# pynbody/topsy

Hardware: AMD Instinct MI355X
Metric: particles/sec splatted to 1024^2 buffer (higher is better)
Workload: dtype f32

## Files before the change

### topsy_amd/csrc/tsp_api.hip

```cpp
#include <stdarg.h>
#include <string.h>

#include <algorithm>
#include <vector>

#include "tsp_internal.h"

namespace tsp {

static thread_local char g_err[1024] = "";

void set_error(const char *fmt, ...) {
    va_list ap;
    va_start(ap, fmt);
    vsnprintf(g_err, sizeof(g_err), fmt, ap);
    va_end(ap);
}

int ensure_array(float **p, int64_t n) {
    if (*p) {
        TSP_HIP(hipFree(*p));
        *p = nullptr;
    }
    if (n > 0) TSP_HIP(hipMalloc((void **)p, (size_t)n * sizeof(float)));
// ... 644 lines not shown
int tsp_content_values(tsp_context *ctx, const int64_t *ranks, int n_ranks, float *out) {
    TSP_REQUIRE(ctx && ranks && out && n_ranks >= 0, TSP_EINVAL, "bad argument");
    TSP_REQUIRE(ctx->sort_keys_alt, TSP_ESTATE, "tsp_content_sort has not been called");
    TSP_HIP(hipSetDevice(ctx->device));
    for (int i = 0; i < n_ranks; ++i) {
        TSP_REQUIRE(ranks[i] >= 0 && ranks[i] < ctx->sorted_count, TSP_EINVAL, "rank %lld outside [0, %lld)",
                    (long long)ranks[i], (long long)ctx->sorted_count);
        uint32_t key;
        TSP_HIP(hipMemcpy(&key, ctx->sort_keys_alt + ranks[i], 4, hipMemcpyDeviceToHost));
        const uint32_t bits = (key & 0x80000000u) ? (key & 0x7fffffffu) : ~key;
        memcpy(&out[i], &bits, 4);
    }
    return TSP_OK;
}

int tsp_get_stats(tsp_context *ctx, tsp_stats *out) {
    TSP_REQUIRE(ctx && out, TSP_EINVAL, "NULL argument");
    *out = ctx->stats;
    return TSP_OK;
}

int tsp_set_option(tsp_context *ctx, const char *name, int64_t value) {
    TSP_REQUIRE(ctx && name, TSP_EINVAL, "NULL argument");
    if (!strcmp(name, "count_fragments")) {
        ctx->count_fragments = value != 0;
        return TSP_OK;
    }
    if (!strcmp(name, "p_small_milli")) {
        TSP_REQUIRE(value >= 0 && value <= 16000, TSP_EINVAL, "p_small out of range (kernel S packs <= 16 texel columns per footprint)");
        ctx->p_small = (float)value * 1e-3f;
        return TSP_OK;
    }
    if (!strcmp(name, "debug_no_raster")) {
        ctx->debug_no_raster = value != 0;
        return TSP_OK;
    }
    if (!strcmp(name, "huge_split") || !strcmp(name, "stream_blocks_per_cu")) {
        TSP_REQUIRE(value >= 0 && value <= 4096, TSP_EINVAL, "%s out of range", name);
        if (name[0] == 'h') ctx->huge_split = (int)value;
        else ctx->stream_blocks_per_cu = (int)value;
        return TSP_OK;
    }
    if (!strcmp(name, "slice_records")) {
        TSP_REQUIRE(value == 0 || (value >= 64 && value <= (1ll << 27)), TSP_EINVAL, "%s: 0 or 64 .. 2^27", name);
        ctx->slice_records = value;
        return TSP_OK;
    }
    if (!strcmp(name, "debug_fail_stage")) {
        TSP_REQUIRE(value >= 0 && value <= 2, TSP_EINVAL, "%s out of range", name);
        ctx->debug_fail_stage = (int)value;
        return TSP_OK;
    }
    if (!strcmp(name, "debug_gather_full_lut")) { ctx->debug_gather_full_lut = value ? 1 : 0; return TSP_OK; }
    if (!strcmp(name, "mid_item_scale_milli")) {
        TSP_REQUIRE(value >= 1 && value <= 100000, TSP_EINVAL, "%s out of range", name);
        ctx->mid_item_scale = (double)value * 1e-3;
        return TSP_OK;
    }
    if (!strcmp(name, "mid_narrow_px_milli")) {
        TSP_REQUIRE(value >= 0 && value <= 64000, TSP_EINVAL, "%s out of range", name);
        ctx->mid_narrow_px = (float)value * 1e-3f;
        return TSP_OK;
    }
    if (!strcmp(name, "mid_item_records")) {
        TSP_REQUIRE(value == 0 || (value >= 64 && value <= 8192 && (value & (value - 1)) == 0), TSP_EINVAL, "%s: 0 or a power of two from 64 to 8192", name);
        ctx->mid_item_records = (int)value;
        return TSP_OK;
    }
    if (!strcmp(name, "stream_batch_chunks")) {
        TSP_REQUIRE(value >= 4 && value <= 4096, TSP_EINVAL, "%s out of range", name);
        ctx->stream_batch_chunks = (int)value;
        return TSP_OK;
    }
    if (!strcmp(name, "huge_band_mib")) {
        TSP_REQUIRE(value >= 0 && value <= (1 << 20), TSP_EINVAL, "%s out of range", name);
        ctx->huge_band_budget = value << 20;
        return TSP_OK;
    }
    if (!strcmp(name, "huge_variant")) {
        TSP_REQUIRE(value >= 1 && value <= 7 && value != 3, TSP_EINVAL, "huge_variant out of range");
        ctx->huge_variant = (int)value;
        return TSP_OK;
    }
    if (!strcmp(name, "reorder_interleave")) {
        TSP_REQUIRE(value >= 0 && value <= 2, TSP_EINVAL, "%s out of range", name);
        ctx->reorder_interleave = (int)value;
        return TSP_OK;
    }
    if (!strcmp(name, "chunk_cull")) {
        ctx->chunk_cull = value != 0;
        return TSP_OK;
    }
    if (!strcmp(name, "overlap_mid_huge")) {
        ctx->overlap_mid_huge = value != 0;
        return TSP_OK;
    }
    if (!strcmp(name, "use_quantity")) {
        ctx->use_quantity = value != 0;
        return TSP_OK;
    }
    if (!strcmp(name, "active_channels")) {
        TSP_REQUIRE((value == 2 || value == 4) && value <= ctx->Ccap, TSP_EINVAL, "bad channel count %lld", (long long)value);
        ctx->C = (int)value;
        return TSP_OK;
    }
    set_error("unknown option '%s'", name);
    return TSP_EINVAL;
}

int tsp_measure_read_bandwidth(tsp_context *ctx, int64_t bytes, int iters, double *gbps_out) {
    TSP_REQUIRE(ctx && gbps_out && bytes > 0 && iters > 0, TSP_EINVAL, "bad argument");
    TSP_HIP(hipSetDevice(ctx->device));
    return measure_read_bandwidth(ctx, bytes, iters, gbps_out);
}

}
```

### topsy_amd/csrc/tsp_gather.hip

```cpp
#include <algorithm>
#include <cmath>
#include <type_traits>

#include "tsp_pipeline.h"

namespace tsp {


template <int T> __device__ __forceinline__ void fmac_quad(float &acc, float rowval, float v) {
    static_assert(T >= 0 && T < 4, "quad lane");
    if (T == 0) asm volatile("v_fmac_f32_dpp %0, %1, %2 " TSP_DPP_QUAD(0) : "+v"(acc) : "v"(rowval), "v"(v));
    if (T == 1) asm volatile("v_fmac_f32_dpp %0, %1, %2 " TSP_DPP_QUAD(1) : "+v"(acc) : "v"(rowval), "v"(v));
    if (T == 2) asm volatile("v_fmac_f32_dpp %0, %1, %2 " TSP_DPP_QUAD(2) : "+v"(acc) : "v"(rowval), "v"(v));
    if (T == 3) asm volatile("v_fmac_f32_dpp %0, %1, %2 " TSP_DPP_QUAD(3) : "+v"(acc) : "v"(rowval), "v"(v));
}
template <int T> __device__ __forceinline__ float mul_quad(float rowval, float v) {
    float r;
    if (T == 0) asm volatile("v_mul_f32_dpp %0, %1, %2 " TSP_DPP_QUAD(0) : "=v"(r) : "v"(rowval), "v"(v));
    if (T == 1) asm volatile("v_mul_f32_dpp %0, %1, %2 " TSP_DPP_QUAD(1) : "=v"(r) : "v"(rowval), "v"(v));
    if (T == 2) asm volatile("v_mul_f32_dpp %0, %1, %2 " TSP_DPP_QUAD(2) : "=v"(r) : "v"(rowval), "v"(v));
    if (T == 3) asm volatile("v_mul_f32_dpp %0, %1, %2 " TSP_DPP_QUAD(3) : "=v"(r) : "v"(rowval), "v"(v));
    return r;
}
__device__ __forceinline__ void fmac_plain(float &acc, float x, float y) {
    asm volatile("v_fmac_f32_e32 %0, %1, %2" : "+v"(acc) : "v"(x), "v"(y));
}

constexpr int PT_ROWS = 66;
constexpr int PT_STRIDE = 65;

constexpr int H2T = 256;

template <int MODE, int NACC, int W, int HR, int OCC, bool CNT>
__global__ __launch_bounds__(H2T, OCC) void splat_huge2_kernel(TileArgs a) {
    constexpr int C = (MODE == TSP_MODE_RGB) ? 4 : 2;
    constexpr int NW = (MODE == TSP_MODE_RGB) ? 2 : 1;
    constexpr int TW = 2 * 64 * W, TH = 2 * HR;
    constexpr int NG = HR / 4;
    static_assert(HR == 16 || HR == 32 || HR == 64, "rows per wave strip");
    typedef typename std::conditional<HR == 64, unsigned long long, unsigned>::type mask_t;
    extern __shared__ __attribute__((aligned(16))) float smem[];
    float *PT = smem;
    float2 *rt_all = reinterpret_cast<float2 *>(smem + ((PT_ROWS * PT_STRIDE + 3) & ~3));

    const int tid = threadIdx.x, lane = tid & 63, wv = __builtin_amdgcn_readfirstlane(tid >> 6);
    const int R = a.cam.R;
    const int tile_id = blockIdx.x / a.split, sp = blockIdx.x % a.split;
    const int tx0 = (tile_id % a.tiles_x) * TW, ty0 = (tile_id / a.tiles_x) * TH;
    for (int i = tid; i < PT_ROWS * PT_STRIDE; i += H2T) {
        const int j = min(i / PT_STRIDE, 63), x = min(i % PT_STRIDE, 63);
        PT[i] = a.mips[j * 64 + x];
    }
    float2 *rt = rt_all + wv * 64;
    const float2 *rt_quad = rt + (lane & 3);
    const int sx = tx0 + 64 * W * (wv & 1), sy = ty0 + HR * (wv >> 1);
    const float sx0 = (float)sx, sx1 = (float)(sx + 64 * W), sy0 = (float)sy, sy1 = (float)(sy + HR);
    float pxc[W];
#pragma unroll
    for (int w = 0; w < W; ++w) pxc[w] = (sx + 64 * w + lane < R) ? (float)(sx + 64 * w + lane) + 0.5f : __builtin_inff();
    const int myrow = lane & (HR - 1);
    const float pyc_own = (sy + myrow < R) ? (float)(sy + myrow) + 0.5f : __builtin_inff();

    constexpr int FOLD_EVERY = TSP_FOLD_EVERY;
    float acc[HR * W][NACC];
#pragma unroll
    for (int p = 0; p < HR * W; ++p)
#pragma unroll
        for (int c = 0; c < NACC; ++c) acc[p][c] = 0.0f;
    unsigned long long n_frag = 0;
    const char *PTb = reinterpret_cast<const char *>(PT);
    __syncthreads();
    if (sx >= R || sy >= R) return;

    const float4 *geom = a.geom;
    const float *wts = a.w;
    unsigned n_rec = (unsigned)a.n_records;
    if (a.hband_count) {
        const int band = ty0 / HBAND_H;
        geom += (size_t)band * a.hband_stride;
        wts += (size_t)band * a.hband_stride * NW;
        n_rec = (unsigned)a.hband_count[band];
    }
    const unsigned n_runs = (n_rec + HDEAL - 1) / HDEAL, usplit = (unsigned)a.split, n_last = max(n_rec, 1u) - 1u;
    const unsigned lane_off = (unsigned)(lane / HDEAL) * usplit * HDEAL + (unsigned)(lane & (HDEAL - 1));
    auto batch_base = [&](unsigned run0) -> unsigned { return (run0 * usplit + sp) * HDEAL; };
    auto fetch = [&](unsigned run0, float4 &g, float &gw1, float &gw2) {
        const unsigned rc = min(batch_base(run0) + lane_off, n_last);
        g = geom[rc];
        gw1 = (NACC >= 2) ? wts[rc * NW] : 0.0f;
        gw2 = (NW == 2) ? wts[rc * NW + 1] : 0.0f;
    };
    float4 g_next; float gw1_next, gw2_next;
    fetch(0, g_next, gw1_next, gw2_next);
    __builtin_amdgcn_s_waitcnt(0x0F70);
    unsigned run0 = 0;
    do {
    int since_fold = 0;
    for (; run0 * usplit < n_runs && since_fold < FOLD_EVERY; run0 += 64 / HDEAL) {
        float4 g = g_next;
        const float gw1 = gw1_next, gw2 = gw2_next;
        if (batch_base(run0) + lane_off >= n_rec) g.z = 0.0f;
        fetch(run0 + 64 / HDEAL, g_next, gw1_next, gw2_next);
        const float g_half = 0.5f * g.z;
        bool hit;
        {
            const float sdx = fmaxf(fmaxf(sx0 - g.x, g.x - sx1), 0.0f), sdy = fmaxf(fmaxf(sy0 - g.y, g.y - sy1), 0.0f);
            hit = g.z > 0.0f && sdx < g_half && sdy < g_half && !(a.disc_k2 > 0.0f && sdx * sdx + sdy * sdy >= a.disc_k2 * g.z * g.z);
        }
        unsigned long long hits = __ballot(hit);
        if (hits == 0ull) continue;
        since_fold += __popcll(hits);
        const float g_invP = 1.0f / g.z;
        const float g_w1 = (MODE == TSP_MODE_RGB) ? gw1 : g.w * gw1;
        constexpr int NH = 64 / HR;
        while (hits) {
            int srcs[NH], n_h = 0;
#pragma unroll
            for (int i = 0; i < NH; ++i) {
                srcs[i] = i ? srcs[0] : 0;
                if (hits) { srcs[i] = __ffsll((long long)hits) - 1; hits &= hits - 1; n_h = i + 1; }
            }
            unsigned long long cov64, chg64, jmp64;
            int r512;
            {
                int src_l = srcs[0];
#pragma unroll
                for (int i = 1; i < NH; ++i) src_l = (lane >= HR * i) ? srcs[i] : src_l;
                const int bp = src_l << 2;
                const float pcy_l = __int_as_float(__builtin_amdgcn_ds_bpermute(bp, __float_as_int(g.y)));
                const float half_l = __int_as_float(__builtin_amdgcn_ds_bpermute(bp, __float_as_int(g_half)));
                const float invP_l = __int_as_float(__builtin_amdgcn_ds_bpermute(bp, __float_as_int(g_invP)));
                const float d = pyc_own - pcy_l;
                const float cv = (__builtin_fabsf(d) < half_l) ? 1.0f : 0.0f;
                const float v = (d + half_l) * invP_l;
                const float tv = __builtin_amdgcn_fmed3f(__builtin_fmaf(v, 64.0f, -0.5f), 0.0f, 63.0f);
                const float fr = __builtin_amdgcn_fractf(tv) * cv;
                const int r = (int)tv;
                const int rprev = __builtin_amdgcn_mov_dpp(r, 0x138, 0xf, 0xf, false);
                r512 = __mul24(r, PT_STRIDE * 4);
                asm volatile("" ::: "memory");
                rt[lane] = make_float2(fr, cv - fr);
                asm volatile("" ::: "memory");
                constexpr unsigned long long ROW0S = (HR == 64) ? 1ull : ((HR == 32) ? 0x0000000100000001ull : 0x0001000100010001ull);
                cov64 = __builtin_amdgcn_fcmpf(__builtin_fabsf(d), half_l, 4 );
                chg64 = __builtin_amdgcn_uicmp((unsigned)r, (unsigned)rprev, 33 ) & cov64 & ~ROW0S;
                jmp64 = __builtin_amdgcn_uicmp((unsigned)r, (unsigned)(rprev + 1), 33 ) & chg64;
            }
            for (int hh = 0; hh < n_h; ++hh) {
            int src = srcs[0];
#pragma unroll
            for (int i = 1; i < NH; ++i) src = (hh == i) ? srcs[i] : src;
            constexpr unsigned long long ROWS = (HR == 64) ? ~0ull : ((1ull << (HR & 63)) - 1ull);
            mask_t covmask = (mask_t)((cov64 >> ((HR * hh) & 63)) & ROWS), chgmask = (mask_t)((chg64 >> ((HR * hh) & 63)) & ROWS),
                   jmpmask = (mask_t)((jmp64 >> ((HR * hh) & 63)) & ROWS);
            const float pcx = __int_as_float(__builtin_amdgcn_readlane(__float_as_int(g.x), src));
            const float half = __int_as_float(__builtin_amdgcn_readlane(__float_as_int(g_half), src));
            const float invP = __int_as_float(__builtin_amdgcn_readlane(__float_as_int(g_invP), src));
            float4 wq;
            wq.x = __int_as_float(__builtin_amdgcn_readlane(__float_as_int(g.w), src));
            wq.y = (NACC >= 2) ? __int_as_float(__builtin_amdgcn_readlane(__float_as_int(g_w1), src)) : 0.0f;
            wq.z = (NACC >= 3) ? __int_as_float(__builtin_amdgcn_readlane(__float_as_int(gw2), src)) : 0.0f;
            wq.w = 0.0f;
            if (NACC >= 2) {
                asm volatile("v_mov_b32 %0, %1" : "=v"(wq.x) : "s"(wq.x));
                asm volatile("v_mov_b32 %0, %1" : "=v"(wq.y) : "s"(wq.y));
                if (NACC >= 3) asm volatile("v_mov_b32 %0, %1" : "=v"(wq.z) : "s"(wq.z));
            }
            const float2 *rt_quad_h = rt_quad + HR * hh;
            if (covmask == 0) continue;
            const mask_t first = covmask & ((mask_t)0 - covmask);
            chgmask &= ~first; jmpmask &= ~first;
            constexpr bool JIT = (HR >= 32);
            constexpr int NRF = JIT ? 2 : NG;
            float2 rowf[NRF];
            if constexpr (JIT) rowf[0] = rt_quad_h[0];
            else {
#pragma unroll
                for (int k = 0; k < NG; ++k) rowf[k] = rt_quad_h[4 * k];
            }
            int caddr[W];
            float fxs[W], gxs[W];
            int ncov_x = 0;
#pragma unroll
            for (int w = 0; w < W; ++w) {
                const float d = pxc[w] - pcx;
                const bool covered = __builtin_fabsf(d) < half;
                const float u = (d + half) * invP;
                const float tu = __builtin_amdgcn_fmed3f(__builtin_fmaf(u, 64.0f, -0.5f), 0.0f, 63.0f);
                caddr[w] = ((int)tu) * 4;
                const float cw = covered ? ((NACC == 1) ? wq.x : 1.0f) : 0.0f;
                const float fr = __builtin_amdgcn_fractf(tu);
                fxs[w] = fr * cw;
                gxs[w] = (1.0f - fr) * cw;
                if (CNT) ncov_x += covered ? 1 : 0;
            }
            float top[W], bot[W];
            float2 nxt[W];
            auto pair_at = [&](int w, int byteoff) -> float2 {
                const float *t = reinterpret_cast<const float *>(PTb + byteoff + caddr[w]);
                return make_float2(t[0], t[1]);
            };
            auto lerp = [&](int w, float2 t) -> float { return __builtin_fmaf(t.y, fxs[w], t.x * gxs[w]); };
            int r_off = __builtin_amdgcn_readlane(r512, (HR == 64 ? __ffsll((long long)covmask) : __ffs((int)covmask)) - 1 + HR * hh);
#pragma unroll
            for (int w = 0; w < W; ++w) {
                top[w] = lerp(w, pair_at(w, r_off)); bot[w] = lerp(w, pair_at(w, r_off + PT_STRIDE * 4));
                nxt[w] = pair_at(w, r_off + 2 * PT_STRIDE * 4);
            }
            auto row_step = [&]() {
                r_off += PT_STRIDE * 4;
#pragma unroll
                for (int w = 0; w < W; ++w) {
                    asm volatile("v_mov_b32 %0, %1\n\tv_mul_f32 %1, %2, %4\n\tv_fmac_f32 %1, %3, %5"
                                 : "=&v"(top[w]), "+v"(bot[w]) : "v"(nxt[w].x), "v"(nxt[w].y), "v"(gxs[w]), "v"(fxs[w]));
                    nxt[w] = pair_at(w, r_off + 2 * PT_STRIDE * 4);
                }
            };
            auto row_change = [&](int , bool skip) {
                if (skip) row_step();
                row_step();
            };
            if constexpr (!JIT) {
#pragma unroll
                for (int k = 0; k < NG; ++k) asm volatile("" : "+v"(rowf[k].x), "+v"(rowf[k].y));
                asm volatile("s_nop 1");
            }
#define TSP_H2_ROW(K, T)                                                                                       \
            {                                                                                                  \
                constexpr int ty_ = 4 * (K) + (T);                                                             \
                if ((chgmask >> ty_) & 1) row_change(ty_, ((jmpmask >> ty_) & 1) != 0);                       \
                _Pragma("unroll") for (int w = 0; w < W; ++w) {                                                \
                    float *ac = acc[ty_ * W + w];                                                              \
                    if (NACC == 1) {                                                                           \
                        fmac_quad<T>(ac[0], rowf[JIT ? ((K) & 1) : (K)].y, top[w]);                                                \
                        fmac_quad<T>(ac[0], rowf[JIT ? ((K) & 1) : (K)].x, bot[w]);                                                \
                    } else {                                                                                   \
                        float kv = mul_quad<T>(rowf[JIT ? ((K) & 1) : (K)].y, top[w]);                                             \
                        fmac_quad<T>(kv, rowf[JIT ? ((K) & 1) : (K)].x, bot[w]);                                                   \
                        fmac_plain(ac[0], kv, wq.x);                                                           \
                        fmac_plain(ac[NACC >= 2 ? 1 : 0], kv, wq.y);                                           \
                        if (NACC >= 3) fmac_plain(ac[NACC - 1], kv, wq.z);                                     \
                    }                                                                                          \
                }                                                                                              \
            }
#define TSP_H2_GROUP(K)                                                                                        \
            if constexpr ((K) < NG) {                                                                          \
                if constexpr (JIT && (K) + 1 < NG) rowf[((K) + 1) & 1] = rt_quad_h[4 * ((K) + 1)];               \
                if (((covmask >> (4 * (K))) & 15) != 0) {                                                    \
                    if constexpr (JIT) asm volatile("" : "+v"(rowf[(K) & 1].x), "+v"(rowf[(K) & 1].y));        \
                    TSP_H2_ROW(K, 0) TSP_H2_ROW(K, 1) TSP_H2_ROW(K, 2) TSP_H2_ROW(K, 3)                          \
                }                                                                                              \
            }
            TSP_H2_GROUP(0) TSP_H2_GROUP(1) TSP_H2_GROUP(2) TSP_H2_GROUP(3)
            TSP_H2_GROUP(4) TSP_H2_GROUP(5) TSP_H2_GROUP(6) TSP_H2_GROUP(7)
            TSP_H2_GROUP(8) TSP_H2_GROUP(9) TSP_H2_GROUP(10) TSP_H2_GROUP(11)
            TSP_H2_GROUP(12) TSP_H2_GROUP(13) TSP_H2_GROUP(14) TSP_H2_GROUP(15)
#undef TSP_H2_GROUP
#undef TSP_H2_ROW
            if (CNT) n_frag += (unsigned long long)(ncov_x * __popcll((unsigned long long)covmask));
#ifdef TSP_H2_DEBUG
            if (CNT && lane == 0) {
                atomicAdd(&a.cnt->n_frag_class[0], 1ull);
                atomicAdd(&a.cnt->n_frag_class[1], (unsigned long long)__popcll((unsigned long long)covmask));
                unsigned long long groups = 0;
                for (int k = 0; k < NG; ++k) groups += (((unsigned long long)covmask >> (4 * k)) & 15ull) ? 1ull : 0ull;
                atomicAdd(&a.cnt->n_frag_class[3], (unsigned long long)__popcll((unsigned long long)chgmask) + (groups << 32));
            }
#endif
            }
        }
    }
    {
        int Rl = R;
        asm volatile("" : "+s"(Rl));
        double *img = a.img + ((size_t)sy * Rl + (sx + lane)) * C;
        asm volatile("" : "+v"(img));
#pragma unroll
        for (int ty = 0; ty < HR; ++ty)
#pragma unroll
            for (int w = 0; w < W; ++w) {
                const int p = ty * W + w, gx = sx + 64 * w + lane, gy = sy + ty;
                if (gx < Rl && gy < Rl) {
                    double *d = img + ((size_t)ty * Rl + 64 * w) * C;
#pragma unroll
                    for (int c = 0; c < NACC; ++c) {
                        if (acc[p][c] != 0.0f) gatomic_add(d + c, acc[p][c]);
                        acc[p][c] = 0.0f;
                    }
                }
            }
    }
    } while (run0 * usplit < n_runs);
    if (CNT) {
        for (int o = 32; o; o >>= 1) n_frag += __shfl_xor((long long)n_frag, o);
        if (lane == 0 && n_frag) { atomicAdd(&a.cnt->n_fragments, n_frag); atomicAdd(&a.cnt->n_frag_class[2], n_frag); }
    }
}

#ifndef TSP_G_OCC1
#define TSP_G_OCC1 8
#define TSP_G_HR1 32
#define TSP_G_OCC2 8
#define TSP_G_OCC3 5
#endif
constexpr int GCHUNK_MAX = 1024;
#ifndef TSP_BIN_PER
#define TSP_BIN_PER 4
#endif
constexpr int G_WIN_TILES = 4096;
constexpr int G_LDS_TILES = 16384;

template <int MODE, int NACC, int HR, int OCC, bool QUAD, bool CNT>
__global__ __launch_bounds__(H2T, OCC) void splat_mid_gather_kernel(TileArgs a) {
    constexpr int C = (MODE == TSP_MODE_RGB) ? 4 : 2;
    constexpr int NW = (MODE == TSP_MODE_RGB) ? 2 : 1;
    constexpr int NG = HR / 4;
    static_assert(HR == 16 || HR == 32, "rows per wave strip");
    extern __shared__ __attribute__((aligned(16))) float smem[];
    constexpr int TSIZE = QUAD ? MIPQ_TOTAL : MIP_TOTAL;
    float *T = smem;
    int *rt_all = reinterpret_cast<int *>(smem + TSIZE);
    typedef const __attribute__((address_space(3))) float LdsF;
    const int T_lds = (int)(unsigned)(unsigned long long)(LdsF *)T;

    const int tid = threadIdx.x, lane = tid & 63, wv = __builtin_amdgcn_readfirstlane(tid >> 6);
    const int R = a.cam.R;
    const int n_items = a.item_base[a.n_tiles];
    if ((int)blockIdx.x * (H2T / 64) >= n_items) return;
    const int item = min((int)blockIdx.x * (H2T / 64) + wv, n_items - 1);
    const bool idle_wave = (int)blockIdx.x * (H2T / 64) + wv >= n_items;
    const int strip = a.item_tile[item];
    const int chunk = item - a.item_base[strip];
    if (QUAD) {
        for (int i = tid; i < MIPQ_TOTAL; i += H2T) {
            const int lvl = i < 1024 ? 0 : (i < 1280 ? 1 : (i < 1344 ? 2 : 3));
            const int hn = 32 >> lvl, k = i - mipq_offset(lvl);
            T[i] = a.mips[mip_offset(lvl) + (k / hn) * (2 * hn) + (k % hn)];
        }
    } else {
        for (int i = tid; i < MIP_TOTAL; i += H2T) T[i] = a.mips[i];
    }
// ... 624 lines not shown
    int rc, n_items = 0;
    ta.n_records = n_mid;
    if ((rc = bin_mid_records<(MODE == TSP_MODE_RGB) ? 2 : 1>(ctx, ta, mid_geom, mid_w, n_mid, 64, HR, pmin, __builtin_inff(), false, &n_items, st))) return rc;
    if (n_items == 0) return TSP_OK;
    const dim3 grid((n_items + H2T / 64 - 1) / (H2T / 64));
    if (quad) {
        if (ta.count_frag) hipLaunchKernelGGL((splat_mid_gather_kernel<MODE, NACC, HR, OCC, true, true>), grid, dim3(H2T), smem, st, ta);
        else hipLaunchKernelGGL((splat_mid_gather_kernel<MODE, NACC, HR, OCC, true, false>), grid, dim3(H2T), smem, st, ta);
    } else {
        if (ta.count_frag) hipLaunchKernelGGL((splat_mid_gather_kernel<MODE, NACC, HR, OCC, false, true>), grid, dim3(H2T), smem, st, ta);
        else hipLaunchKernelGGL((splat_mid_gather_kernel<MODE, NACC, HR, OCC, false, false>), grid, dim3(H2T), smem, st, ta);
    }
    TSP_HIP(hipGetLastError());
    return TSP_OK;
}

template <int MODE, int NACC, int HR, int OCC>
static int launch_narrow_gather_kernel(tsp_context *ctx, TileArgs ta, const float4 *mid_geom, const float *mid_w, long long n_mid, float pmax, hipStream_t st) {
    const bool quad = ctx->lut_mirror_symmetric && !ctx->debug_gather_full_lut;
    const size_t smem = (size_t)(quad ? NQ_LINES * 32 : MIP_TOTAL + 64) * sizeof(float) + (H2T / 64) * 4 * HR * sizeof(int);
    int rc, n_items = 0;
    ta.n_records = n_mid;
    if ((rc = bin_mid_records<(MODE == TSP_MODE_RGB) ? 2 : 1>(ctx, ta, mid_geom, mid_w, n_mid, NSW, HR, 0.0f, pmax, true, &n_items, st))) return rc;
    if (n_items == 0) return TSP_OK;
    const dim3 grid((n_items + H2T / 64 - 1) / (H2T / 64));
    if (quad) {
        if (ta.count_frag) hipLaunchKernelGGL((splat_narrow_gather_kernel<MODE, NACC, HR, OCC, true, true>), grid, dim3(H2T), smem, st, ta);
        else hipLaunchKernelGGL((splat_narrow_gather_kernel<MODE, NACC, HR, OCC, true, false>), grid, dim3(H2T), smem, st, ta);
    } else {
        if (ta.count_frag) hipLaunchKernelGGL((splat_narrow_gather_kernel<MODE, NACC, HR, OCC, false, true>), grid, dim3(H2T), smem, st, ta);
        else hipLaunchKernelGGL((splat_narrow_gather_kernel<MODE, NACC, HR, OCC, false, false>), grid, dim3(H2T), smem, st, ta);
    }
    TSP_HIP(hipGetLastError());
    return TSP_OK;
}

template <int MODE>
static int launch_mid_gather_mode(tsp_context *ctx, TileArgs ta, bool second_channel, const float4 *mid_geom, const float *mid_w, long long n_mid, hipStream_t st) {
    TSP_REQUIRE(n_mid < (1ll << 28), TSP_EINVAL, "%lld mid footprints in one launch (kernel G indexes its work items with 32 bits; run_pipeline slices the list)", n_mid);
    const float split = ctx->mid_narrow_px;
    int rc;
    if (split > 0.0f) {
        if (MODE == TSP_MODE_RGB) rc = launch_narrow_gather_kernel<MODE, 3, 16, TSP_G_OCC3>(ctx, ta, mid_geom, mid_w, n_mid, split, st);
        else if (second_channel) rc = launch_narrow_gather_kernel<MODE, 2, 16, TSP_G_OCC2>(ctx, ta, mid_geom, mid_w, n_mid, split, st);
        else rc = launch_narrow_gather_kernel<MODE, 1, TSP_G_HR1, TSP_G_OCC1>(ctx, ta, mid_geom, mid_w, n_mid, split, st);
        if (rc) return rc;
        if (split >= P_BILINEAR) return TSP_OK;
    }
    if (MODE == TSP_MODE_RGB) return launch_mid_gather_kernel<MODE, 3, 16, TSP_G_OCC3>(ctx, ta, mid_geom, mid_w, n_mid, split, st);
    if (second_channel) return launch_mid_gather_kernel<MODE, 2, 16, TSP_G_OCC2>(ctx, ta, mid_geom, mid_w, n_mid, split, st);
    return launch_mid_gather_kernel<MODE, 1, TSP_G_HR1, TSP_G_OCC1>(ctx, ta, mid_geom, mid_w, n_mid, split, st);
}

int launch_mid_gather(tsp_context *ctx, TileArgs ta, int mode, bool second_channel, const float4 *mid_geom, const float *mid_w,
                      long long n_mid, hipStream_t st) {
    switch (mode) {
        case TSP_MODE_WEIGHTED: return launch_mid_gather_mode<TSP_MODE_WEIGHTED>(ctx, ta, second_channel, mid_geom, mid_w, n_mid, st);
        case TSP_MODE_DEPTH: return launch_mid_gather_mode<TSP_MODE_DEPTH>(ctx, ta, true, mid_geom, mid_w, n_mid, st);
        case TSP_MODE_RGB: return launch_mid_gather_mode<TSP_MODE_RGB>(ctx, ta, true, mid_geom, mid_w, n_mid, st);
    }
    set_error("bad mode %d", mode);
    return TSP_EINVAL;
}

template <int MODE, int NACC, int W, int HR, int OCC>
static int launch_huge2(tsp_context *ctx, TileArgs ta, long long n_huge) {
    TSP_REQUIRE(ta.n_records < (1ll << 31), TSP_EINVAL, "%lld deferred footprints in one render block (the tile-gather kernels index them with 32 bits)", ta.n_records);
    const size_t smem = (size_t)((PT_ROWS * PT_STRIDE + 3) & ~3) * sizeof(float) + (H2T / 64) * 64 * sizeof(float2);
    const int tw = 2 * 64 * W, th = 2 * HR;
    const int htiles_x = (ctx->R + tw - 1) / tw, htiles_y = (ctx->R + th - 1) / th;
    const int htiles = htiles_x * htiles_y;
    const long long batches = (n_huge + 63) / 64;
    int split = ctx->huge_split;
    if (split <= 0) {
        split = std::max(1, (ctx->cu_count * 128 + htiles - 1) / htiles);
        if (n_huge < (1ll << 16)) split = std::max(32, (int)((long long)split * n_huge >> 16));
        else if (HR == 32 && NACC == 1) split = n_huge >= 2000000 ? split : (n_huge >= 1000000 ? (split * 3) / 4 : split / 2);
        else if (HR == 16 && NACC == 1) split = std::max(1, split / 2);
        else if (HR == 16 && NACC == 2 && n_huge < 1000000) split = std::max(1, split / 2);
    }
    split = (int)std::min<long long>(split, std::max<long long>(batches, 1));
    ta.split = split;
    ta.tiles_x = htiles_x;
    if (ta.count_frag) hipLaunchKernelGGL((splat_huge2_kernel<MODE, NACC, W, HR, OCC, true>), dim3(htiles * split), dim3(H2T), smem, ctx->stream, ta);
    else hipLaunchKernelGGL((splat_huge2_kernel<MODE, NACC, W, HR, OCC, false>), dim3(htiles * split), dim3(H2T), smem, ctx->stream, ta);
    TSP_HIP(hipGetLastError());
    return TSP_OK;
}

template <int MODE>
static int launch_gather_mode(tsp_context *ctx, TileArgs ta, bool second_channel, const float4 *huge_geom, const float *huge_w,
                              long long n_huge) {
    hipStream_t st = ctx->stream;
    int rc = TSP_OK;
    if (n_huge > 0) {
        ta.geom = huge_geom; ta.w = huge_w; ta.n_records = n_huge;
        TSP_REQUIRE(n_huge < (1ll << 31), TSP_EINVAL, "%lld deferred footprints in one render block (the tile-gather kernel indexes them with 32 bits)", n_huge);
        if ((rc = bin_huge_records<(MODE == TSP_MODE_RGB) ? 2 : 1>(ctx, ta, huge_geom, huge_w, n_huge))) return rc;
        if (MODE == TSP_MODE_RGB) {
            if (ctx->huge_variant == 4) rc = launch_huge2<MODE, 3, 1, 16, 4>(ctx, ta, n_huge);
            else rc = launch_huge2<MODE, 3, 1, 16, 5>(ctx, ta, n_huge);
        } else if (second_channel) {
            if (ctx->huge_variant == 4) rc = launch_huge2<MODE, 2, 1, 16, 4>(ctx, ta, n_huge);
            else rc = launch_huge2<MODE, 2, 1, 16, 7>(ctx, ta, n_huge);
        }
        else if (ctx->huge_variant == 2) rc = launch_huge2<MODE, 1, 1, 32, 6>(ctx, ta, n_huge);
        else if (ctx->huge_variant == 4) rc = launch_huge2<MODE, 1, 1, 16, 7>(ctx, ta, n_huge);
        else if (ctx->huge_variant == 5) rc = launch_huge2<MODE, 1, 1, 16, 8>(ctx, ta, n_huge);
        else if (ctx->huge_variant == 6) rc = launch_huge2<MODE, 1, 1, 32, 7>(ctx, ta, n_huge);
        else if (ctx->huge_variant == 7 || (ctx->huge_variant == 1 && n_huge >= 250000)) rc = launch_huge2<MODE, 1, 1, 32, 8>(ctx, ta, n_huge);
        else rc = launch_huge2<MODE, 1, 1, 16, 8>(ctx, ta, n_huge);
        if (rc) return rc;
    }
    TSP_HIP(hipEventRecord(ctx->ev[10], st));
    return TSP_OK;
}

int launch_gather_kernels(tsp_context *ctx, TileArgs ta, int mode, bool second_channel, const float4 *huge_geom, const float *huge_w,
                          long long n_huge) {
    switch (mode) {
        case TSP_MODE_WEIGHTED: return launch_gather_mode<TSP_MODE_WEIGHTED>(ctx, ta, second_channel, huge_geom, huge_w, n_huge);
        case TSP_MODE_DEPTH: return launch_gather_mode<TSP_MODE_DEPTH>(ctx, ta, true, huge_geom, huge_w, n_huge);
        case TSP_MODE_RGB: return launch_gather_mode<TSP_MODE_RGB>(ctx, ta, true, huge_geom, huge_w, n_huge);
    }
    set_error("bad mode %d", mode);
    return TSP_EINVAL;
}

}
```

### topsy_amd/csrc/tsp_internal.h

```cpp
#pragma once
#include <hip/hip_runtime.h>
#include <stdint.h>

#include <vector>
#include <stdio.h>
#include <string>

#include "../../include/topsy_splat.h"
#include "tsp_math.h"

namespace tsp {

void set_error(const char *fmt, ...);

#define TSP_HIP(call)                                                                          \
    do {                                                                                       \
        hipError_t e_ = (call);                                                                \
        if (e_ != hipSuccess) {                                                                \
            tsp::set_error("%s failed: %s (%s:%d)", #call, hipGetErrorString(e_), __FILE__, __LINE__); \
            return TSP_EHIP;                                                                   \
        }                                                                                      \
    } while (0)

#define TSP_REQUIRE(cond, code, ...)       \
// ... 17 lines not shown

constexpr int BOUNDS_BLOCK = 512;

struct Record {
    float pcx, pcy, P, w0, w1;
};
struct Record4 {
    float pcx, pcy, P, w0, w1, w2;
};

struct Counters {
    unsigned long long n_small, n_mid, n_huge, n_culled, n_fragments, huge_count, next_chunk, mid_odd_weights;
    unsigned long long n_frag_class[4];
};

struct Workspace {
    void *mid_geom = nullptr, *mid_w = nullptr;
    int64_t mid_capacity = 0;
    void *huge_geom = nullptr, *huge_w = nullptr;
    int64_t huge_capacity = 0;
    void *hband_geom = nullptr, *hband_w = nullptr;
    int *hband_count = nullptr;
    int64_t hband_stride = 0; int hband_bands = 0;
    void *mband_geom = nullptr, *mband_w = nullptr;
    int *mband_count = nullptr;
    long long *mband_base = nullptr;
    int64_t mband_capacity = 0;
    int mtile_capacity = 0;
    int64_t mitem_capacity = 0;
    int *mitem_tile = nullptr, *mitem_base = nullptr;
    int64_t chunk_capacity = 0;
    float4 *block_bounds = nullptr;
    int64_t bounds_capacity = 0;
    bool bounds_valid = false;
    int *alive_list = nullptr;
    unsigned long long *cull_info = nullptr;
    int64_t *range_prefix = nullptr;
    int64_t range_capacity = 0;
    int *count_diff = nullptr;
    int *count_band = nullptr;
};

}

struct tsp_context {
    int device = 0;
    int R = 0, C = 0, Ccap = 0;
    bool use_quantity = true;
    hipStream_t stream = nullptr;
    hipStream_t stream2 = nullptr;
    hipEvent_t ev[12] = {};
    float *image = nullptr;
    double *image64 = nullptr;
    double *image64_entry = nullptr;
    float *mips = nullptr;
    bool have_mips = false;
    bool lut_mirror_symmetric = false;
    bool lut_zero_outside_disc = false;
    tsp::Particles p;
    tsp::Counters *counters = nullptr;
    tsp::Workspace ws;
    uint8_t *out8 = nullptr;
    float *outf = nullptr;
    float *lut = nullptr;
    int lut_capacity = 0;
    float *lut2d = nullptr;
    int lut2d_n = 0;
    void *scratch = nullptr;
    size_t scratch_bytes = 0;
    uint32_t *sort_keys = nullptr, *sort_keys_alt = nullptr;
    void *sort_tmp = nullptr;
    size_t sort_tmp_bytes = 0;
    int64_t sort_capacity = 0, sorted_count = 0;
    tsp_stats stats = {};
    std::vector<int64_t> cell_offsets;
    int cell_bits = 0;
    float cell_lo[3] = {0, 0, 0}, cell_width[3] = {0, 0, 0};
    std::vector<int64_t> strata_offsets;
    uint32_t kernel_attr_done = 0;
    bool count_fragments = false;
    float p_small = 16.0f;
    int64_t huge_band_budget = 6ll << 30;
    int huge_variant = 1;
    int huge_split = 0;
    int reorder_interleave = 2;
    int stream_blocks_per_cu = 0;
    int debug_gather_full_lut = 0;
    double mid_item_scale = 0.35;
    float mid_narrow_px = 64.0f;
    int mid_item_records = 0;
    int stream_batch_chunks = 8;
    bool chunk_cull = true;
    int64_t chunk_culled_particles = 0;
    bool overlap_mid_huge = false;
    int64_t slice_records = 0;
    int debug_fail_stage = 0;
    int stream_occ[3][2] = {};
    bool debug_no_raster = false;
    int cu_count = 256;
    void *comm = nullptr;
    int n_ranks = 1, rank = 0;
    bool image_is_reduced = false;
};

namespace tsp {
struct DeviceScratch {
    void *p = nullptr;
    DeviceScratch() = default;
    DeviceScratch(const DeviceScratch &) = delete;
    DeviceScratch &operator=(const DeviceScratch &) = delete;
    ~DeviceScratch() { if (p) (void)hipFree(p); }
    hipError_t alloc(size_t bytes) { return hipMalloc(&p, bytes ? bytes : 16); }
    template <typename T> T *as() const { return static_cast<T *>(p); }
    void *release() { void *q = p; p = nullptr; return q; }
    void reset(void *q) { if (p) (void)hipFree(p); p = q; }
};

int launch_generic(tsp_context *ctx, const Camera &cam, const int64_t *d_ranges, int n_ranges,
                   int64_t total, int mode, int rule);
int launch_pipeline(tsp_context *ctx, const Camera &cam, const int64_t *h_starts, const int64_t *h_lens,
                    int n_ranges, int64_t total, int mode);
int launch_colormap_scalar(tsp_context *ctx, const float *d_img, int64_t npix, int C, const float *d_lut,
                           int n_lut, float vmin, float vmax, int log_scale, int weighted, uint8_t *d_out);
int launch_colormap_rgb(tsp_context *ctx, const float *d_img, int64_t npix, int C, float vmin, float vmax,
                        float gamma, uint8_t *d_out8, float *d_outf);
int launch_colormap_bivariate(tsp_context *ctx, const float *d_img, int64_t npix, int C, float vmin, float vmax,
                             float dvmin, float dvmax, int log_scale, int weighted, uint8_t *d_out);
int generate_synthetic(tsp_context *ctx, int64_t n_total, int64_t first, int64_t count, uint64_t seed,
                       float h_cap, int with_quantity, int with_rgb);
int reorder_spatial(tsp_context *ctx, int n_strata, uint64_t seed, int64_t *perm_out);
int ensure_weights(tsp_context *ctx, bool rgb);
int ensure_block_bounds(tsp_context *ctx);
int measure_read_bandwidth(tsp_context *ctx, int64_t bytes, int iters, double *gbps_out);
int launch_image_convert(tsp_context *ctx, bool to_float);
int tile_periodic(tsp_context *ctx, int n, const float *h_offsets, const float *h_weights);
int content_sort(tsp_context *ctx, int kind, float scale, int64_t *n_finite, int64_t *n_nonpositive);
int ensure_array(float **p, int64_t n);
}
```

Measured before the change: 19.72 billion.

## Hand-write huge-particle row walk as a single inline-asm state machine

Adds an inline-assembly row walker for the huge-particle splat kernel, used in the single-channel, W=1, OCC=8 case with 16- or 32-row strips. It rotates the top, bottom and next lerp rows through a four-state register rotation, branches on scalar coverage and change masks, and interleaves LDS reads with DPP FMACs, all to cut compiler-generated moves and waitcnts in the inner loop. A runtime knob h2_walk is added and defaults to on. In exchange it adds much larger code size, scalar branches, and fragile hand-managed register and lgkmcnt ordering.

After: 20.79 billion (median of 6 runs). +5.4%, better.

```diff
diff --git a/topsy_amd/csrc/tsp_api.hip b/topsy_amd/csrc/tsp_api.hip
--- a/topsy_amd/csrc/tsp_api.hip
+++ b/topsy_amd/csrc/tsp_api.hip
@@ -750,6 +750,11 @@
         ctx->huge_variant = (int)value;
         return TSP_OK;
     }
+    if (!strcmp(name, "h2_walk")) {
+        TSP_REQUIRE(value == 0 || value == 1, TSP_EINVAL, "%s out of range", name);
+        ctx->h2_walk = (int)value;
+        return TSP_OK;
+    }
     if (!strcmp(name, "reorder_interleave")) {
         TSP_REQUIRE(value >= 0 && value <= 2, TSP_EINVAL, "%s out of range", name);
         ctx->reorder_interleave = (int)value;
diff --git a/topsy_amd/csrc/tsp_gather.hip b/topsy_amd/csrc/tsp_gather.hip
--- a/topsy_amd/csrc/tsp_gather.hip
+++ b/topsy_amd/csrc/tsp_gather.hip
@@ -26,13 +26,135 @@
     asm volatile("v_fmac_f32_e32 %0, %1, %2" : "+v"(acc) : "v"(x), "v"(y));
 }
 
+#define H2A_S_(x) #x
+#define H2A_S(x) H2A_S_(x)
+#define H2A_TOP0 "%[r0]"
+#define H2A_TOP1 "%[r1]"
+#define H2A_TOP2 "%[r0]"
+#define H2A_TOP3 "%[r1]"
+#define H2A_BOT0 "%[r1]"
+#define H2A_BOT1 "%[r0]"
+#define H2A_BOT2 "%[r1]"
+#define H2A_BOT3 "%[r0]"
+#define H2A_NEXT0 "1"
+#define H2A_NEXT1 "2"
+#define H2A_NEXT2 "3"
+#define H2A_NEXT3 "0"
+#define H2A_STEP0 ""
+#define H2A_STEP1 ""
+#define H2A_STEP2 ""
+#define H2A_STEP3 "v_add_u32 %[va], 0x410, %[va]\n\t"
+#define H2A_DPP(q) " quad_perm:[" #q "," #q "," #q "," #q "] row_mask:0xf bank_mask:0xf\n\t"
+#define H2A_ROW(S, t, q, p)                                                                                    \
+    "v_fmac_f32_dpp %[a" #t "], %[gy" #p "], " H2A_TOP##S H2A_DPP(q)                                           \
+    "v_fmac_f32_dpp %[a" #t "], %[fy" #p "], " H2A_BOT##S H2A_DPP(q)
+#define H2A_TROW(S, t, q, p)                                                                                   \
+    "s_bitcmp1_b32 %[chg], " #t "\n\t"                                                                         \
+    "s_cbranch_scc1 .Lh2c" #S "_" #t "_%=\n"                                                                   \
+    ".Lh2r" #S "_" #t "_%=:\n\t" H2A_ROW(S, t, q, p)
+#define H2A_GROUP(S, K, p, pn, t0, t1, t2, t3)                                                                 \
+    ".Lh2g" #S "_" #K "_%=:\n\t"                                                                               \
+    "ds_read_b32 %[fy" #pn "], %[rt] offset:32*(" #K "+1)\n\t"                                                 \
+    "ds_read_b32 %[gy" #pn "], %[rt] offset:32*(" #K "+1)+4\n\t"                                               \
+    "s_and_b32 %[tmp], %[cov], 15<<(4*" #K ")\n\t"                                                             \
+    "s_cbranch_scc0 .Lh2k" #S "_" #K "_%=\n\t"                                                                 \
+    "s_waitcnt lgkmcnt(2)\n\t"                   \
+    "s_and_b32 %[tmp], %[chg], 15<<(4*" #K ")\n\t"                                                             \
+    "s_cbranch_scc1 .Lh2s" #S "_" #K "_%=\n\t"                                                                 \
+    H2A_ROW(S, t0, 0, p) H2A_ROW(S, t1, 1, p) H2A_ROW(S, t2, 2, p) H2A_ROW(S, t3, 3, p)
+#define H2A_GROUP_LAST(S, K, p, t0, t1, t2, t3)                                                                \
+    ".Lh2g" #S "_" #K "_%=:\n\t"                                                                               \
+    "s_and_b32 %[tmp], %[cov], 15<<(4*" #K ")\n\t"                                                             \
+    "s_cbranch_scc0 .Lh2end_%=\n\t"                                                                            \
+    "s_waitcnt lgkmcnt(0)\n\t"                                                                                 \
+    "s_and_b32 %[tmp], %[chg], 15<<(4*" #K ")\n\t"                                                             \
+    "s_cbranch_scc1 .Lh2s" #S "_" #K "_%=\n\t"                                                                 \
+    H2A_ROW(S, t0, 0, p) H2A_ROW(S, t1, 1, p) H2A_ROW(S, t2, 2, p) H2A_ROW(S, t3, 3, p)                        \
+    "s_branch .Lh2end_%=\n"
+#define H2A_SLOW(S, K, N, p, t0, t1, t2, t3)                                                                   \
+    ".Lh2s" #S "_" #K "_%=:\n\t"                                                                               \
+    H2A_TROW(S, t0, 0, p) H2A_TROW(S, t1, 1, p) H2A_TROW(S, t2, 2, p) H2A_TROW(S, t3, 3, p)                    \
+    "s_branch .Lh2" #N "_%=\n"
+#define H2A_SKIP(S, K, N)                                                                                      \
+    ".Lh2k" #S "_" #K "_%=:\n\t"                                                                               \
+    "s_lshr_b32 %[tmp], %[cov], 4*(" #K "+1)\n\t"                                                              \
+    "s_cbranch_scc0 .Lh2end_%=\n\t"                                                                            \
+    "s_branch .Lh2" #N "_%=\n"
+#define H2A_CHG(S, t)                                                                                          \
+    ".Lh2c" #S "_" #t "_%=:\n\t"                                                                               \
+    "s_waitcnt lgkmcnt(0)\n\t"                                                                                 \
+    "v_mul_f32 " H2A_TOP##S ", %[nx], %[gx]\n\t"                                                               \
+    "v_fmac_f32 " H2A_TOP##S ", %[ny], %[fx]\n\t"                                                              \
+    "ds_read_b32 %[nx], %[va] offset:260*(" #S "+1)\n\t"                                                       \
+    "ds_read_b32 %[ny], %[va] offset:260*(" #S "+1)+4\n\t"                                                     \
+    H2A_STEP##S                                                                                                \
+    "s_bitcmp1_b32 %[jmp], " #t "\n\t"                                                                         \
+    "s_cbranch_scc0 .Lh2r" H2A_NEXT##S "_" #t "_%=\n\t"                                                        \
+    "s_bitset0_b32 %[jmp], " #t "\n\t"                                                                         \
+    "s_branch .Lh2c" H2A_NEXT##S "_" #t "_%=\n"
+#define H2A_CHG4(S, a, b, c, d) H2A_CHG(S, a) H2A_CHG(S, b) H2A_CHG(S, c) H2A_CHG(S, d)
+#define H2A_STATE16(S)                                                                                         \
+    H2A_GROUP(S, 0, 0, 1, 0, 1, 2, 3) H2A_GROUP(S, 1, 1, 0, 4, 5, 6, 7) H2A_GROUP(S, 2, 0, 1, 8, 9, 10, 11)     \
+    H2A_GROUP_LAST(S, 3, 1, 12, 13, 14, 15)                                                                    \
+    H2A_SLOW(S, 0, g##S##_1, 0, 0, 1, 2, 3) H2A_SLOW(S, 1, g##S##_2, 1, 4, 5, 6, 7)                            \
+    H2A_SLOW(S, 2, g##S##_3, 0, 8, 9, 10, 11) H2A_SLOW(S, 3, end, 1, 12, 13, 14, 15)                           \
+    H2A_SKIP(S, 0, g##S##_1) H2A_SKIP(S, 1, g##S##_2) H2A_SKIP(S, 2, g##S##_3)                                 \
+    H2A_CHG4(S, 0, 1, 2, 3) H2A_CHG4(S, 4, 5, 6, 7) H2A_CHG4(S, 8, 9, 10, 11) H2A_CHG4(S, 12, 13, 14, 15)
+#define H2A_STATE32(S)                                                                                         \
+    H2A_GROUP(S, 0, 0, 1, 0, 1, 2, 3) H2A_GROUP(S, 1, 1, 0, 4, 5, 6, 7) H2A_GROUP(S, 2, 0, 1, 8, 9, 10, 11)     \
+    H2A_GROUP(S, 3, 1, 0, 12, 13, 14, 15) H2A_GROUP(S, 4, 0, 1, 16, 17, 18, 19)                                \
+    H2A_GROUP(S, 5, 1, 0, 20, 21, 22, 23) H2A_GROUP(S, 6, 0, 1, 24, 25, 26, 27)                                \
+    H2A_GROUP_LAST(S, 7, 1, 28, 29, 30, 31)                                                                    \
+    H2A_SLOW(S, 0, g##S##_1, 0, 0, 1, 2, 3) H2A_SLOW(S, 1, g##S##_2, 1, 4, 5, 6, 7)                            \
+    H2A_SLOW(S, 2, g##S##_3, 0, 8, 9, 10, 11) H2A_SLOW(S, 3, g##S##_4, 1, 12, 13, 14, 15)                      \
+    H2A_SLOW(S, 4, g##S##_5, 0, 16, 17, 18, 19) H2A_SLOW(S, 5, g##S##_6, 1, 20, 21, 22, 23)                    \
+    H2A_SLOW(S, 6, g##S##_7, 0, 24, 25, 26, 27) H2A_SLOW(S, 7, end, 1, 28, 29, 30, 31)                         \
+    H2A_SKIP(S, 0, g##S##_1) H2A_SKIP(S, 1, g##S##_2) H2A_SKIP(S, 2, g##S##_3) H2A_SKIP(S, 3, g##S##_4)         \
+    H2A_SKIP(S, 4, g##S##_5) H2A_SKIP(S, 5, g##S##_6) H2A_SKIP(S, 6, g##S##_7)                                 \
+    H2A_CHG4(S, 0, 1, 2, 3) H2A_CHG4(S, 4, 5, 6, 7) H2A_CHG4(S, 8, 9, 10, 11) H2A_CHG4(S, 12, 13, 14, 15)      \
+    H2A_CHG4(S, 16, 17, 18, 19) H2A_CHG4(S, 20, 21, 22, 23) H2A_CHG4(S, 24, 25, 26, 27) H2A_CHG4(S, 28, 29, 30, 31)
+#define H2A_HEAD                                                                                               \
+    "ds_read_b32 %[nx], %[va]\n\t"                                                                             \
+    "ds_read_b32 %[ny], %[va] offset:4\n\t"                                                                    \
+    "ds_read_b32 %[fy0], %[rt]\n\t"                                                                            \
+    "ds_read_b32 %[gy0], %[rt] offset:4\n"
+#define H2A_TAIL ".Lh2end_%=:\n\t" "s_waitcnt lgkmcnt(0)"
+#define H2A_A4(a, i, j, k, l) [a##i] "+v"(acc[i][0]), [a##j] "+v"(acc[j][0]), [a##k] "+v"(acc[k][0]), [a##l] "+v"(acc[l][0])
+#define H2A_OPERANDS                                                                                           \
+    [r0] "+v"(top), [r1] "+v"(bot), [nx] "=&v"(nx), [ny] "=&v"(ny), [fy0] "=&v"(fy0), [gy0] "=&v"(gy0),         \
+    [fy1] "=&v"(fy1), [gy1] "=&v"(gy1), [va] "+v"(va), [jmp] "+s"(jmp), [tmp] "=&s"(tmp)
+#define H2A_INPUTS [gx] "v"(gx), [fx] "v"(fx), [rt] "v"(rt), [cov] "s"(cov), [chg] "s"(chg)
+
+template <int HR>
+__device__ __forceinline__ void h2_walk_asm(float (&acc)[HR][1], float top, float bot, float gx, float fx, int va, int rt,
+                                            unsigned cov, unsigned chg, unsigned jmp) {
+    float nx, ny, fy0, gy0, fy1, gy1;
+    unsigned tmp;
+    if constexpr (HR == 16) {
+        asm volatile(H2A_HEAD H2A_STATE16(0) H2A_STATE16(1) H2A_STATE16(2) H2A_STATE16(3) H2A_TAIL
+                     : H2A_A4(a, 0, 1, 2, 3), H2A_A4(a, 4, 5, 6, 7), H2A_A4(a, 8, 9, 10, 11), H2A_A4(a, 12, 13, 14, 15),
+                       H2A_OPERANDS
+                     : H2A_INPUTS
+                     : "memory", "scc");
+    } else {
+        static_assert(HR == 32, "asm row walk: 64 x 16 and 64 x 32 strips");
+        asm volatile(H2A_HEAD H2A_STATE32(0) H2A_STATE32(1) H2A_STATE32(2) H2A_STATE32(3) H2A_TAIL
+                     : H2A_A4(a, 0, 1, 2, 3), H2A_A4(a, 4, 5, 6, 7), H2A_A4(a, 8, 9, 10, 11), H2A_A4(a, 12, 13, 14, 15),
+                       H2A_A4(a, 16, 17, 18, 19), H2A_A4(a, 20, 21, 22, 23), H2A_A4(a, 24, 25, 26, 27), H2A_A4(a, 28, 29, 30, 31),
+                       H2A_OPERANDS
+                     : H2A_INPUTS
+                     : "memory", "scc");
+    }
+}
+
 constexpr int PT_ROWS = 66;
 constexpr int PT_STRIDE = 65;
 
 constexpr int H2T = 256;
 
-template <int MODE, int NACC, int W, int HR, int OCC, bool CNT>
+template <int MODE, int NACC, int W, int HR, int OCC, bool CNT, bool AW>
 __global__ __launch_bounds__(H2T, OCC) void splat_huge2_kernel(TileArgs a) {
+    static_assert(!AW || (NACC == 1 && W == 1 && (HR == 16 || HR == 32)), "asm row walk: single channel, 64 x 16 / 64 x 32 strips");
     constexpr int C = (MODE == TSP_MODE_RGB) ? 4 : 2;
     constexpr int NW = (MODE == TSP_MODE_RGB) ? 2 : 1;
     constexpr int TW = 2 * 64 * W, TH = 2 * HR;
@@ -194,6 +316,18 @@
                 gxs[w] = (1.0f - fr) * cw;
                 if (CNT) ncov_x += covered ? 1 : 0;
             }
+            if constexpr (AW) {
+                typedef const __attribute__((address_space(3))) float LdsF;
+                const int r_off = __builtin_amdgcn_readlane(r512, __ffs((int)covmask) - 1 + HR * hh);
+                auto lerp_at = [&](int byteoff) -> float {
+                    const float *t = reinterpret_cast<const float *>(PTb + byteoff + caddr[0]);
+                    return __builtin_fmaf(t[1], fxs[0], t[0] * gxs[0]);
+                };
+                const float t0 = lerp_at(r_off), t1 = lerp_at(r_off + PT_STRIDE * 4);
+                const int va = (int)(unsigned)(unsigned long long)(LdsF *)PT + r_off + 2 * PT_STRIDE * 4 + caddr[0];
+                const int rtq = (int)(unsigned)(unsigned long long)(LdsF *)(const float *)rt_quad_h;
+                h2_walk_asm<HR>(acc, t0, t1, gxs[0], fxs[0], va, rtq, (unsigned)covmask, (unsigned)chgmask, (unsigned)jmpmask);
+            } else {
             float top[W], bot[W];
             float2 nxt[W];
             auto pair_at = [&](int w, int byteoff) -> float2 {
@@ -257,6 +391,7 @@
             TSP_H2_GROUP(12) TSP_H2_GROUP(13) TSP_H2_GROUP(14) TSP_H2_GROUP(15)
 #undef TSP_H2_GROUP
 #undef TSP_H2_ROW
+            }
             if (CNT) n_frag += (unsigned long long)(ncov_x * __popcll((unsigned long long)covmask));
 #ifdef TSP_H2_DEBUG
             if (CNT && lane == 0) {
@@ -1047,8 +1182,12 @@
     split = (int)std::min<long long>(split, std::max<long long>(batches, 1));
     ta.split = split;
     ta.tiles_x = htiles_x;
-    if (ta.count_frag) hipLaunchKernelGGL((splat_huge2_kernel<MODE, NACC, W, HR, OCC, true>), dim3(htiles * split), dim3(H2T), smem, ctx->stream, ta);
-    else hipLaunchKernelGGL((splat_huge2_kernel<MODE, NACC, W, HR, OCC, false>), dim3(htiles * split), dim3(H2T), smem, ctx->stream, ta);
+    constexpr bool AW_BUILT = NACC == 1 && W == 1 && OCC == 8;
+    if (AW_BUILT && ctx->h2_walk) {
+        if (ta.count_frag) hipLaunchKernelGGL((splat_huge2_kernel<MODE, NACC, W, HR, OCC, true, AW_BUILT>), dim3(htiles * split), dim3(H2T), smem, ctx->stream, ta);
+        else hipLaunchKernelGGL((splat_huge2_kernel<MODE, NACC, W, HR, OCC, false, AW_BUILT>), dim3(htiles * split), dim3(H2T), smem, ctx->stream, ta);
+    } else if (ta.count_frag) hipLaunchKernelGGL((splat_huge2_kernel<MODE, NACC, W, HR, OCC, true, false>), dim3(htiles * split), dim3(H2T), smem, ctx->stream, ta);
+    else hipLaunchKernelGGL((splat_huge2_kernel<MODE, NACC, W, HR, OCC, false, false>), dim3(htiles * split), dim3(H2T), smem, ctx->stream, ta);
     TSP_HIP(hipGetLastError());
     return TSP_OK;
 }
diff --git a/topsy_amd/csrc/tsp_internal.h b/topsy_amd/csrc/tsp_internal.h
--- a/topsy_amd/csrc/tsp_internal.h
+++ b/topsy_amd/csrc/tsp_internal.h
@@ -123,6 +123,7 @@
     float p_small = 16.0f;
     int64_t huge_band_budget = 6ll << 30;
     int huge_variant = 1;
+    int h2_walk = 1;
     int huge_split = 0;
     int reorder_interleave = 2;
     int stream_blocks_per_cu = 0;
```
